# febrianrachmadi/dep-gan-im

Hardware: AMD Instinct MI355X
Metric: 2D slices/sec (G+2D+GP train step), 256x256x1 fp32 (higher is better)
Workload: dtype f32; 1 GPU; DEP-GAN-IM twoCritics canonical train step (critic-Y2 + critic-DEM + G update, WGAN-GP), batch 32 per GPU, 256x256x1; per_gpu_batch=32, global_batch=32, parallelism=dp1

## Files before the change

dep_gan_im_amd/csrc/common.h:

```cpp
#pragma once
#include <hip/hip_runtime.h>
#include <stdint.h>
#include <stddef.h>

typedef float f32x2 __attribute__((ext_vector_type(2)));
typedef float f32x4 __attribute__((ext_vector_type(4)));
typedef float f32x16 __attribute__((ext_vector_type(16)));

struct TView {
  float* p;
  long sB, sY, sX;
};

static inline TView make_view(float* p, int H, int W, int C) {
  TView v;
  v.p = p;
  v.sX = C;
  v.sY = (long)W * C;
  v.sB = (long)H * W * C;
  return v;
}
static inline TView make_view_slice(float* p, int H, int W, int Ctot, int c0) {
  TView v = make_view(p, H, W, Ctot);
  v.p = p + c0;
// ... 32 lines not shown
}

struct Epilogue {
  const float* bias;
  const float* scale;
  const float* shift;
  const float* film_mul;
  const float* film_add;
  int film_ld;
  TView out_pre;
  TView res;
  TView mask;
  int relu;
  int accumulate;
  TView pool;
  const float* head_w;
  const float* head_b;
  float* head_out;
  int head_tanh, head_skip_out;
};

struct ConvArgs {
  TView in;
  TView out;
  const float* w;
  int B, H, W, Cin, Cout;
  Epilogue ep;
  long wsT, wsI, wsO;
  int flip;
  int vec4;
// ... 238 lines not shown
```

dep_gan_im_amd/csrc/igemm_epilogue.inc:

```
#ifndef EPI_PRE_SYNC
#define EPI_PRE_SYNC __syncthreads()
#define EPI_PRE_SYNC_DEFAULTED
#endif
  EPI_PRE_SYNC;
  constexpr int CP = NT + 4;
#ifdef EPI_ES_BASE
  float* es = EPI_ES_BASE;
#else
  float* es = smem + wv * (64 * CP);
#endif
  constexpr int NQ = (MF == 32) ? 4 : 1, CSTEP = (MF == 32) ? 8 : 4;
#if defined(EPI_STAGE)
  EPI_STAGE;
  (void)es;
#elif !defined(EPI_PHASED)
#pragma unroll
  for (int mt = 0; mt < MT; ++mt)
#pragma unroll
    for (int g = 0; g < NQ; ++g) {
      f32x4 q4;
#pragma unroll
      for (int k = 0; k < 4; ++k) q4[k] = acc[mt][4 * g + k];
      *reinterpret_cast<f32x4*>(es + (MF * mt + r) * CP + CSTEP * g + 4 * h) = q4;
    }
// ... 56 lines not shown
      const unsigned lo = __builtin_amdgcn_readfirstlane((unsigned)u), hi = __builtin_amdgcn_readfirstlane((unsigned)(u >> 32));
      return __builtin_amdgcn_make_buffer_rsrc((void*)(((unsigned long long)hi << 32) | lo), 0, 0x7FFFFFFF, 0x00020000);
    };
    const int lo_out = 4 * (pl0 * (int)a.out.sX + co);
    const int lo_pre = has_pre ? 4 * (pl0 * (int)e.out_pre.sX + co) : 0;
    const int lo_res = has_res ? 4 * (pl0 * (int)e.res.sX + co) : 0;
    const int lo_msk = has_msk ? 4 * (pl0 * (int)e.mask.sX + co) : 0;
    const __amdgpu_buffer_rsrc_t r_out = mk(a.out.p + out_goff + view_off(a.out, b, oyw, tx0));
    const __amdgpu_buffer_rsrc_t r_pre = mk(has_pre ? e.out_pre.p + view_off(e.out_pre, b, oyw, tx0) : a.out.p);
    const __amdgpu_buffer_rsrc_t r_res = mk(has_res ? e.res.p + view_off(e.res, b, oyw, tx0) : a.out.p);
    const __amdgpu_buffer_rsrc_t r_msk = mk(has_msk ? e.mask.p + view_off(e.mask, b, oyw, tx0) : a.out.p);
    const __amdgpu_buffer_rsrc_t r_pool =
        mk(has_pool ? e.pool.p + view_off(e.pool, b, oyw >> 1, tx0 >> 1) : a.out.p);
    const int lo_pool = has_pool ? 4 * ((pl0 >> 1) * (int)e.pool.sX + co) : 0;
    const int sY_pool = 4 * (int)e.pool.sY, sX_pool = 4 * (int)e.pool.sX;
    f32x4 vrow = {0.f, 0.f, 0.f, 0.f};
#ifdef EPI_HEAD
#ifdef EPI_CLASS
    const bool has_head = EPI_HEAD && (EPI_CT ? EpiC::head : (e.head_out != nullptr));
#else
    const bool has_head = EPI_HEAD && e.head_out != nullptr;
#endif
    f32x4 hw4 = {0.f, 0.f, 0.f, 0.f};
    if (has_head) hw4 = *reinterpret_cast<const f32x4*>(e.head_w + co);
    const bool skip_out = has_head && e.head_skip_out != 0;
#else
    constexpr bool has_head = false, skip_out = false;
#endif
    typedef int i32x4 __attribute__((ext_vector_type(4)));
    auto ld = [&](const __amdgpu_buffer_rsrc_t& r, int voff, int soff) {
// ... 82 lines not shown
#undef EPI_DPP
        hkeep_out = ((lane & 7) == p) ? d : hkeep_out;
      }
#endif
      if (has_pool) {
        if ((py & 1) == 0) {
          vrow = v;
        } else {
          f32x4 m;
#pragma unroll
          for (int k = 0; k < 4; ++k) {
            const float t = dg_vmax(vrow[k], v[k]);
            m[k] = dg_vmax(t, __shfl_xor(t, LPP, 64));
          }
          if (ok && (pl0 & 1) == 0) st(r_pool, lo_pool, (py >> 1) * sY_pool + (px0 >> 1) * sX_pool, m);
        }
      }
    }
  }
#ifdef EPI_HEAD
  if (EPI_HEAD && a.ep.head_out != nullptr && n0 < a.Cout) {
    const int ph = lane & 7, plh = lane >> 3;
    const int pyh = (ph & 1) + 2 * (ph >> 2), pxh = ((ph >> 1) & 1) * 8 + plh;
    const int yh = oyw + pyh, xh = tx0 + pxh;
    if (yh < a.H && xh < a.W) {
      const float t = hkeep_out + a.ep.head_b[0];
      a.ep.head_out[((long)b * a.H + yh) * a.W + xh] = a.ep.head_tanh ? tanhf(t) : t;
    }
  }
#endif
// ... 5 lines not shown
```

dep_gan_im_amd/csrc/model.h:

```cpp
#pragma once
#include <string.h>

#include <map>
#include <string>
#include <type_traits>
#include <vector>

#include "../../include/depgan.h"
#include "common.h"
#include "bf16s.h"
#include "bf16s_train.h"
#include "deconv_fwd.h"
#include "noise.h"
#include "ops.h"
#include "train_ops.h"

struct PInfo {
  std::string name;
  int shape[4];
  int ndim;
  size_t off, size;
  bool trainable;
};

// ... 41 lines not shown
  int col_mul = -1, col_add = -1;
  TView in, out;
  TViewH hin = null_view_h(), hout = null_view_h(), hu = null_view_h();
  unsigned char* hdec = nullptr;
  int cat_deconv = -1;
  TView din, dout;
  TView in_mask;
  Tn u;
  Tn raw;
  float *bmean = nullptr, *bvar = nullptr, *bs = nullptr, *bt = nullptr, *brstd = nullptr;
  float *cA = nullptr, *cB = nullptr, *cC = nullptr, *sums = nullptr;
  int skip_of = -1;
  TView pool_dsrc;
  TView pool_skipgrad;
  TView pool_dst;
};

struct DLayer {
  std::string name;
  int KS, Cin, Cout, H, W;
  bool pool;
  ConvPlan pf, pb;
  ConvPlan pf16, pb16;
  bool has16f = false, has16b = false;
};

struct DNet {
  Net net;
  PackJob* pack_jobs = nullptr;
  int n_pack = 0;
// ... 38 lines not shown
  float* dheads = nullptr;
  Tn attr;
  Tn du_tmp;
  float* dpre = nullptr;
  float* zbuf = nullptr;

  DNet d[2];
  std::vector<DLayer> dl;
  int NB3 = 0;
  float* d_in = nullptr;
  Tn d_act[11];
  Tn d_pool[11];
  Tn d_dz[11];
  Tn d_dpool[11];
  Tn d_ufull;
  float *d_t9 = nullptr, *d_out = nullptr;
  float* g0 = nullptr;
  float* coefs = nullptr;
  float *norms = nullptr, *gp = nullptr;

  depgan_allreduce_fn ar_fn = nullptr;
  void* ar_user = nullptr;
  int world = 1;
  void* rccl_comm = nullptr;
  long rccl_issued = 0;
  int device = 0;
  bool winograd = true;
  bool head_fused = true;
  bool wgrad_bf16 = true;
  float* host_stats = nullptr;
// ... 42 lines not shown
  float *n_dl = nullptr, *n_dflat = nullptr, *n_dl1 = nullptr, *n_da0 = nullptr, *n_dl0 = nullptr;

  bool dbg_capture = false;
  float* dbg_mixed[11] = {nullptr, nullptr, nullptr, nullptr, nullptr, nullptr, nullptr, nullptr, nullptr, nullptr, nullptr};
  bool dbg_mixed_valid = false;

  bool h_ready = false, h_valid = false;
  bool fwd_only_bf16 = false;
  bool bf16s_head_fused = true;
  bool h_17_skipped = false;
  bool g_update_bf16 = false;
  bool hu_ready = false, hu_valid = false;

  bool critic16_bf16 = false;

  bool prof_on = false;
  std::vector<ProfRec> recs;
};

struct ProfScope {
  depgan_ctx* c;
  bool live;
  ProfScope(depgan_ctx* c_, int klass, double flops, const char* label = "", double bytes = 0.0,
            const char* kernel = "")
      : c(c_), live(c_ && c_->prof_on) {
    if (!live) return;
    ProfRec r;
    r.klass = klass;
    r.flops = flops;
    r.bytes = bytes;
// ... 184 lines not shown
```

dep_gan_im_amd/csrc/model.hip:

```cpp
#include "model.h"

#include <dlfcn.h>
#include <float.h>
#include <math.h>
#include <stdlib.h>
#include <stdarg.h>
#include <stdio.h>
#include <string.h>

static thread_local char g_err[1024] = "";
void dg_set_error(const char* fmt, ...) {
  va_list ap;
  va_start(ap, fmt);
  vsnprintf(g_err, sizeof(g_err), fmt, ap);
  va_end(ap);
}
const char* dg_get_error() { return g_err; }

void Net::add(const std::string& name, std::vector<int> shape, bool trainable) {
  PInfo pi;
  pi.name = name;
  pi.ndim = (int)shape.size();
  pi.size = 1;
  for (int i = 0; i < 4; ++i) {
// ... 447 lines not shown
      L.dout = d.view();
      if (r.per_sample() > maxFilm) maxFilm = r.per_sample();
      cur = L.out;
    } else if (e.kind == G_POOL) {
      const GLayer& Pc = c->gl[i - 1];
      Cat& ct = cats[e.name];
      Tn p, dp;
      DGCHECK(talloc(c, &p, B, H / 2, W / 2, Pc.Cout));
      DGCHECK(galloc(&dp, B, H / 2, W / 2, Pc.Cout));
      L.Cin = L.Cout = Pc.Cout;
      L.skip_of = i - 1;
      L.out = p.view();
      L.pool_dsrc = dp.view();
      L.pool_skipgrad = fwd_only ? null_view() : ct.grad.slice(ct.co_deconv);
      L.pool_dst = Pc.dout;
      H /= 2;
      W /= 2;
      cur = L.out;
    } else if (e.kind == G_DECONV) {
      L.pf = plan_conv(c, 1, L.Cin, L.Cout);
      L.pb = plan_conv(c, 1, L.Cout, L.Cin);
      for (int t = 0; t < 4; ++t) {
        DGCHECK(dmalloc(c, &L.wpf[t], L.pf.packedFloats));
        if (!fwd_only) DGCHECK(dmalloc(c, &L.wpb[t], L.pb.packedFloats));
      }
      L.pbf = plan_conv(c, 1, 4 * L.Cout, L.Cin);
      if (!fwd_only && dg_plan_mfma(L.pb) && L.pbf.family == L.pb.family && L.pbf.planes == L.pb.planes && (L.Cout % L.pb.CK) == 0 &&
          L.pbf.packedFloats == 4 * L.pb.packedFloats)
        DGCHECK(dmalloc(c, &L.wpb_all, L.pbf.packedFloats));
      Cat& ct = cats[e.aux];
// ... 45 lines not shown
    L.H = H;
    L.W = W;
    L.pf = plan_conv(c, L.KS, L.Cin, L.Cout, 96, H, W);
    L.pb = plan_conv(c, L.KS, L.Cout, L.Cin, 96, H, W);
    if (c->cfg.bf16_mfma) {
      L.pf16 = dg_plan_conv_bf16_n16(L.KS, L.Cin, L.Cout);
      L.pb16 = dg_plan_conv_bf16_n16(L.KS, L.Cout, L.Cin);
      L.has16f = dg_plan_mfma(L.pf) && !dg_plan_bf16(L.pf) && dg_plan_bf16(L.pf16);
      L.has16b = l > 0 && dg_plan_mfma(L.pb) && !dg_plan_bf16(L.pb) && dg_plan_bf16(L.pb16);
    }
    DGCHECK(talloc(c, &c->d_act[l], c->NB3, H, W, L.Cout));
    DGCHECK(talloc(c, &c->d_dz[l], c->NB3, H, W, L.Cout));
    if (L.pool) {
      DGCHECK(talloc(c, &c->d_pool[l], c->NB3, H / 2, W / 2, L.Cout));
      DGCHECK(talloc(c, &c->d_dpool[l], c->NB3, H / 2, W / 2, L.Cout));
      H /= 2;
      W /= 2;
    }
  }
  const int HW = H * W;
  DGCHECK(talloc(c, &c->d_ufull, B, H0, W0, 16));
  DGCHECK(dmalloc(c, &c->d_in, (size_t)c->NB3 * H0 * W0));
  DGCHECK(dmalloc(c, &c->d_t9, (size_t)c->NB3 * HW));
  DGCHECK(dmalloc(c, &c->d_out, (size_t)c->NB3));
  DGCHECK(dmalloc(c, &c->g0, (size_t)2 * B * H0 * W0));
  DGCHECK(dmalloc(c, &c->coefs, 8));
  DGCHECK(dmalloc(c, &c->norms, (size_t)B));
  DGCHECK(dmalloc(c, &c->gp, 4));
  const float hc[4] = {-1.0f / B, 1.0f / B, 1.0f, 1.0f};
  HIPCHECK(hipMemcpy(c->coefs, hc, sizeof(hc), hipMemcpyHostToDevice));
// ... 130 lines not shown
        jobs.push_back(j);
      }
      if (D.wpb16[l]) {
        DGCHECK(dg_pack_job(L.pb16, D.W[l], L.Cin, L.Cout, 0, 1, 1, nullptr, D.wpb16[l], 0, &j));
        jobs.push_back(j);
      }
    }
    D.n_pack = (int)jobs.size();
    D.pack_blocks = dg_pack_layout(jobs.data(), D.n_pack);
    DGCHECK(upload_table(c, jobs, &D.pack_jobs));
  }
  ProfScope ps(c, 2, 0.0, "pack weights");
  return dg_pack_weights_batch(D.pack_jobs, D.n_pack, D.pack_blocks, c->st);
}

int g_forward(depgan_ctx* c, const float* x, const float* z, int n, bool store_u) {
  {
    ProfScope ps(c, 2, 0.0, "noise mlp fwd");
    DGCHECK(dg_noise_fwd(c->np, z, c->na, n, c->st));
  }
  bool pooled_by_conv = false, head_by_conv = false;
  for (size_t i = 0; i < c->gl.size(); ++i) {
    GLayer& L = c->gl[i];
    if (L.kind == G_CONV || L.kind == G_FILM) {
      ConvArgs a = conv_args((i == 0) ? make_view(const_cast<float*>(x), L.H, L.W, L.Cin) : L.in, L.out,
                             n, L.H, L.W, L.Cin, L.Cout);
      g_layer_epilogue(&a.ep, L, c->na.heads, L.in);
      if (L.kind == G_FILM && store_u) a.ep.out_pre = L.u.view();
      conv_set_weights(&a, L.pf, L.wpf[0], L.Wt, L.Cin, L.Cout);
      if (dg_plan_mfma(L.pf) && g_pool_follows(c->gl, i)) a.ep.pool = c->gl[i + 1].out;
      pooled_by_conv = a.ep.pool.p != nullptr;
      head_by_conv = false;
      if (L.kind == G_CONV && i + 1 < c->gl.size() && c->gl[i + 1].kind == G_HEAD && c->cfg.nc_out == 1 &&
          c->head_fused && dg_conv_igemm_head_supported(L.pf, a)) {
        const GLayer& Hd = c->gl[i + 1];
        a.ep.head_w = Hd.Wt; a.ep.head_b = Hd.b; a.ep.head_out = c->attr.p;
        a.ep.head_tanh = 1;
        a.ep.head_skip_out = (!store_u && !c->dbg_capture) ? 1 : 0;
        head_by_conv = true;
      }
      DGCHECK(conv_launch(c, L.pf, a, 3));
    } else if (L.kind == G_POOL) {
      if (pooled_by_conv && L.skip_of == (int)i - 1) continue;
      ProfScope ps(c, 2, 0.0, "maxpool");
      DGCHECK(dg_maxpool(c->gl[L.skip_of].out, L.out, n, L.H / 2, L.W / 2, L.Cout, c->st));
// ... 37 lines not shown
      DGCHECK(dg_sum(c->dpre, (size_t)P, L.db, c->scratch, c->scratchFloats, c->st));
      DGCHECK(dg_head_bwd(c->dpre, L.Wt, L.in.p, L.din.p, P, L.Cin, c->st));
    } else if (L.kind == G_CONV) {
      DGCHECK(g_conv_bn_bwd(c, L, (size_t)i, x, L.dout, null_view(), n));
    } else if (L.kind == G_FILM) {
      TView du = make_view(c->du_tmp.p, L.H, L.W, L.Cout);
      {
        ProfScope ps(c, 2, 0.0, "film bwd");
        DGCHECK(dg_film_bwd(L.dout.p, L.u.p, c->na.heads + L.col_mul, c->na.heads + L.col_add, 1024, du.p,
                            c->dheads + L.col_mul, c->dheads + L.col_add, n, (long)L.H * L.W, L.Cout, c->scratch,
                            c->scratchFloats, c->st));
      }
      DGCHECK(g_conv_bn_bwd(c, L, (size_t)i, x, du, L.dout, n));
    } else if (L.kind == G_POOL) {
      ProfScope ps(c, 2, 0.0, "unpool+mask");
      DGCHECK(dg_unpool_mask(L.pool_dsrc, c->gl[L.skip_of].out, L.pool_skipgrad, L.pool_dst, n, L.H / 2, L.W / 2,
                             L.Cout, c->st));
    } else if (L.kind == G_DECONV) {
      DGCHECK(deconv_wgrad_all(c, L, L.in, L.dout, n, L.s, c->raw_all + (L.dW - c->g.G), L.s, L.db, L.dbeta));
      DGCHECK(deconv_bwd_data(c, L, L.dout, n));
    }
  }
  return g_backward_finish(c, z, n);
}

int g_backward_finish(depgan_ctx* c, const float* z, int n) {
  {
    if (!c->g_gamma_jobs) {
      std::vector<GammaJob> jobs;
      int blk = 0;
      for (size_t i = 0; i < c->gl.size(); ++i) {
        const GLayer& L = c->gl[i];
// ... 20 lines not shown
}

static const ConvPlan& d_plan_f(const depgan_ctx* c, int l) {
  return (c->critic16_bf16 && c->dl[l].has16f) ? c->dl[l].pf16 : c->dl[l].pf;
}
static const float* d_panel_f(const depgan_ctx* c, const DNet& D, int l) {
  return (c->critic16_bf16 && c->dl[l].has16f) ? D.wpf16[l] : D.wpf[l];
}
static const ConvPlan& d_plan_b(const depgan_ctx* c, int l) {
  return (c->critic16_bf16 && c->dl[l].has16b) ? c->dl[l].pb16 : c->dl[l].pb;
}
static const float* d_panel_b(const depgan_ctx* c, const DNet& D, int l) {
  return (c->critic16_bf16 && c->dl[l].has16b) ? D.wpb16[l] : D.wpb[l];
}

static int d_forward(depgan_ctx* c, DNet& D, const float* img, long s0, int N) {
  const int H0 = c->cfg.height, W0 = c->cfg.width;
  for (int l = 0; l < 11; ++l) {
    const DLayer& L = c->dl[l];
    ConvArgs a = conv_args((l == 0) ? make_view(const_cast<float*>(img), H0, W0, 1) : d_in_view(c, l, s0),
                           view_offset(c->d_act[l].view(), s0), N, L.H, L.W, L.Cin, L.Cout);
    a.ep.bias = D.b[l];
    a.ep.relu = 1;
    const ConvPlan& pf = d_plan_f(c, l);
    conv_set_weights(&a, pf, d_panel_f(c, D, l), D.W[l], L.Cin, L.Cout);
    if (dg_plan_mfma(pf) && L.pool && !((L.H | L.W) & 1))
      a.ep.pool = view_offset(c->d_pool[l].view(), s0);
    DGCHECK(conv_launch(c, pf, a, L.KS));
    if (L.pool && !a.ep.pool.p) {
      ProfScope ps(c, 2, 0.0, "maxpool");
      DGCHECK(dg_maxpool(a.out, view_offset(c->d_pool[l].view(), s0), N, L.H / 2, L.W / 2, L.Cout, c->st));
    }
  }
  const DLayer& T = c->dl[10];
  const int HW = T.H * T.W;
  ProfScope ps(c, 2, 0.0, "critic tail fwd");
  return dg_critic_tail_fwd(c->d_act[10].p + s0 * c->d_act[10].per_sample(), D.w9, D.b9, D.wd, D.bd,
                            c->d_t9 + s0 * HW, c->d_out + s0, N, HW, 256, c->st);
}

static int d_backward_chain(depgan_ctx* c, DNet& D, long s0, int N, const float* coefs, int per, long img_s0,
                            int img_n, float* g0_out) {
// ... 6 lines not shown
  }
  for (int l = 10; l >= 1; --l) {
    const DLayer& L = c->dl[l];
    const DLayer& Pv = c->dl[l - 1];
    ConvArgs a = conv_args(view_offset(c->d_dz[l].view(), s0), null_view(), N, L.H, L.W, L.Cout, L.Cin);
    a.w = d_panel_b(c, D, l);
    if (Pv.pool) {
      a.out = view_offset(c->d_dpool[l - 1].view(), s0);
    } else {
      a.out = view_offset(c->d_dz[l - 1].view(), s0);
      a.ep.mask = view_offset(c->d_act[l - 1].view(), s0);
    }
    DGCHECK(conv_launch(c, d_plan_b(c, l), a, L.KS));
    if (Pv.pool) {
      ProfScope ps(c, 2, 0.0, "unpool+mask");
      DGCHECK(dg_unpool_mask(a.out, view_offset(c->d_act[l - 1].view(), s0), null_view(),
                             view_offset(c->d_dz[l - 1].view(), s0), N, Pv.H / 2, Pv.W / 2, Pv.Cout, c->st));
    }
  }
  if (img_n > 0) {
    const DLayer& L = c->dl[0];
    ConvArgs a = conv_args(view_offset(c->d_dz[0].view(), s0 + img_s0), make_view(g0_out, L.H, L.W, 1),
                           img_n, L.H, L.W, L.Cout, 1);
    conv_set_weights_bwd(&a, dg_plan_direct(), nullptr, D.W[0], L.Cin, L.Cout);
    DGCHECK(conv_launch(c, dg_plan_direct(), a, L.KS));
  }
  return DG_OK;
}

int net_adam(depgan_ctx* c, Net& n, float gscale) {
  n.adam_t += 1;
  const double b1 = c->cfg.beta1, b2 = c->cfg.beta2;
// ... 30 lines not shown
  n.decay_bits = (unsigned*)b;
  n.gnorm = (double*)g;
  return dalloc_fills_done();
}

static int critic_enqueue(depgan_ctx* c, int which, const float* y2, const float* x, const float* z, const float* ep) {
  if (c->cfg.nc_out != 1) { dg_set_error("the WGAN-GP closures need nc_out == 1"); return DG_ERR_ARG; }
  DNet& D = c->d[which];
  const int B = c->cfg.batch, H0 = c->cfg.height, W0 = c->cfg.width;
  const long HW0 = (long)H0 * W0;
  DGCHECK(g_forward_only(c, x, z));
  {
    ProfScope ps(c, 2, 0.0, "critic inputs");
    DGCHECK(dg_critic_inputs(y2, x, c->cfg.nicg, c->attr.p, ep, c->d_in, B, HW0, which, c->st));
  }
  DGCHECK(d_forward(c, D, c->d_in, 0, 3 * B));
  if (c->dbg_capture) {
    for (int l = 0; l < 11; ++l) {
      const size_t per = c->d_act[l].per_sample();
      if (!c->dbg_mixed[l]) {
        DGCHECK(dmalloc(c, &c->dbg_mixed[l], (size_t)B * per));
        DGCHECK(dalloc_fills_done());
      }
      HIPCHECK(hipMemcpyAsync(c->dbg_mixed[l], c->d_act[l].p + (size_t)2 * B * per, (size_t)B * per * sizeof(float),
                              hipMemcpyDeviceToDevice, c->st));
    }
    c->dbg_mixed_valid = true;
  }
  DGCHECK(d_backward_chain(c, D, 0, 3 * B, c->coefs, B, 2 * B, B, c->g0));
  float* u0 = c->d_in + 2 * B * HW0;
  {
    ProfScope ps(c, 2, 0.0, "gp norms+u0");
    DGCHECK(dg_gp_u0(c->g0, u0, c->norms, nullptr, c->cfg.delta, B, HW0, c->scratch, c->scratchFloats, c->st));
  }
  for (int l = 0; l < 11; ++l) {
    const DLayer& L = c->dl[l];
    TView act = view_offset(c->d_act[l].view(), 2 * B);
    ConvArgs a = conv_args((l == 0) ? make_view(u0, H0, W0, 1) : d_in_view(c, l, 2 * B),
                           L.pool ? make_view(c->d_ufull.p, L.H, L.W, L.Cout) : act, B, L.H, L.W, L.Cin, L.Cout);
    a.ep.mask = act;
    conv_set_weights(&a, d_plan_f(c, l), d_panel_f(c, D, l), D.W[l], L.Cin, L.Cout);
    DGCHECK(conv_launch(c, d_plan_f(c, l), a, L.KS));
    if (L.pool) {
      ProfScope ps(c, 2, 0.0, "gather pool");
      DGCHECK(dg_gather_pool(a.out, act, view_offset(c->d_pool[l].view(), 2 * B), B, L.H / 2, L.W / 2, L.Cout,
                             c->st));
    }
  }
  for (int l = 0; l < 11; ++l) {
    const DLayer& L = c->dl[l];
    TView xin = (l == 0) ? make_view(c->d_in, H0, W0, 1) : d_in_view(c, l, 0);
    const ColSum cs = {2 * B, nullptr, D.db[l], nullptr};
    DGCHECK(wgrad_full(c, L.KS, xin, c->d_dz[l].view(), 3 * B, L.H, L.W, L.Cin, L.Cout, nullptr, D.dW[l], nullptr, 0,
                       0, &cs));
  }
  {
    ProfScope ps(c, 2, 0.0, "critic tail wgrad+stats");
    const DLayer& T = c->dl[10];
    const int HW = T.H * T.W;
    DGCHECK(dg_critic_tail_wgrad(c->d_act[10].p, D.w9, D.b9, D.wd, c->coefs, B, 1, 0, D.dw9, D.db9, D.dwd, D.dbd,
                                 c->scratch, c->scratchFloats, 2 * B, HW, 256, c->st));
// ... 7 lines not shown

static int g_eval_enqueue(depgan_ctx* c, const float* x, const float* y2, const float* z, bool train,
                          float* stats_dev) {
  const int B = c->cfg.batch, H0 = c->cfg.height, W0 = c->cfg.width;
  const long HW0 = (long)H0 * W0, P = (long)B * HW0;
  if (train) {
    if (c->g_update_bf16) DGCHECK(g_forward_train_bf16s(c, x, z));
    else DGCHECK(g_forward(c, x, z, B, true));
  } else {
    DGCHECK(g_forward_only(c, x, z));
  }
  {
    ProfScope ps(c, 2, 0.0, "fake_y2");
    DGCHECK(dg_add_ch0(x, c->cfg.nicg, c->attr.p, c->fake_y2, P, c->st));
  }
  DGCHECK(d_forward(c, c->d[0], c->fake_y2, 0, B));
  DGCHECK(d_forward(c, c->d[1], c->attr.p, B, B));
  {
    ProfScope ps(c, 2, 0.0, "g loss sums");
    DGCHECK(dg_sum_groups_consts(c->d_out, stats_dev, 2, B, 6, (float)B, (float)P, c->st));
    DGCHECK(dg_gloss_sums(x, c->cfg.nicg, y2, c->attr.p, c->cfg.im_thresh, stats_dev + 2, P, c->scratch,
                                  c->scratchFloats, c->st));
  }
  if (train) {
    DGCHECK(d_backward_chain(c, c->d[0], 0, B, c->coefs + 2, B, 0, B, c->g0));
    DGCHECK(d_backward_chain(c, c->d[1], B, B, c->coefs + 2, B, 0, B, c->g0 + P));
    {
      ProfScope ps(c, 2, 0.0, "g dpre");
      DGCHECK(dg_g_dpre(x, c->cfg.nicg, y2, c->attr.p, c->g0, c->g0 + P, c->dpre, B, P, c->st));
    }
    if (c->g_update_bf16) DGCHECK(g_backward_bf16s(c, x, z, B));
    else DGCHECK(g_backward(c, x, z, B));
// ... 167 lines not shown
    dg_set_error("depgan_create: need batch >= 1, height/width multiples of 16, nicg in {1,2}");
    return DG_ERR_ARG;
  }
  depgan_ctx* c = new depgan_ctx();
  c->cfg = *cfg;
  if (hipGetDevice(&c->device) != hipSuccess) c->device = 0;
  {
    const char* e = getenv("DEPGAN_WGRAD_BF16");
    c->wgrad_bf16 = !(e && atoi(e) == 0);
    const char* hf = getenv("DEPGAN_HEAD_FUSED");
    c->head_fused = !(hf && atoi(hf) == 0);
    const char* hfs = getenv("DEPGAN_BF16S_HEAD_FUSED");
    c->bf16s_head_fused = !(hfs && atoi(hfs) == 0);
    const char* wn = getenv("DEPGAN_WINOGRAD");
    c->winograd = !(wn && atoi(wn) == 0);
  }
  if (c->cfg.nc_out == 0) c->cfg.nc_out = 1;
  if (c->cfg.nc_out < 1 || c->cfg.nc_out > DEPGAN_MAX_HEAD_CLASSES) {
    dg_set_error("depgan_create: nc_out must be 1 (DEP-GAN) or in [2, %d] (DEP-UResNet classes), not %d",
                 DEPGAN_MAX_HEAD_CLASSES, c->cfg.nc_out);
    delete c;
    return DG_ERR_ARG;
  }
  c->infer_only = c->cfg.bf16_mfma && c->cfg.nc_out >= 2;
  c->train_bn = c->cfg.nc_out != 1 && !c->infer_only;
  memset(c->last_sums, 0, sizeof(c->last_sums));
  int rc = build_generator(c);
  if (rc == DG_OK && !c->train_bn && !c->infer_only) rc = build_critics(c);
  if (rc == DG_OK && c->train_bn) rc = uresnet_build(c);
  if (rc == DG_OK && c->infer_only)
// ... 204 lines not shown
  if (pipe != 0 && pipe != 1) {
    dg_set_error("depgan_set_critic16_pipe: pipe must be 0 (fp32) or 1 (bf16), got %d", pipe);
    return DG_ERR_ARG;
  }
  DGCHECK(infer_refuse(c, "depgan_set_critic16_pipe"));
  if (pipe == 1 && (!c->cfg.bf16_mfma || c->dl.empty())) {
    dg_set_error("depgan_set_critic16_pipe: the bf16 pipe for the critics' 16-channel layers needs a context created with "
                 "bf16_mfma = 1 (and critics: nc_out = 1)");
    return DG_ERR_UNSUPPORTED;
  }
  c->critic16_bf16 = pipe == 1;
  return DG_OK;
}
int depgan_get_critic16_pipe(depgan_ctx* c) { return (c && c->critic16_bf16) ? 1 : 0; }

int depgan_g_forward(depgan_ctx* c, const float* x, const float* z, float* out, int n) {
  if (n < 1 || n > c->cfg.batch) { dg_set_error("g_forward: n must be in [1, batch]"); return DG_ERR_ARG; }
  if (c->cfg.nc_out != 1) return uresnet_predict(c, x, z, out, n);
  DGCHECK(g_forward(c, x, z, n, false));
  HIPCHECK(hipMemcpyAsync(out, c->attr.p, (size_t)n * c->cfg.height * c->cfg.width * sizeof(float),
                          hipMemcpyDeviceToDevice, c->st));
  return DG_OK;
}

int depgan_d_forward(depgan_ctx* c, int net, const float* img, float* out, int n) {
  DGCHECK(infer_refuse(c, "depgan_d_forward"));
  if (net != DEPGAN_NET_D_Y2 && net != DEPGAN_NET_D_DEM) { dg_set_error("d_forward: not a critic id"); return DG_ERR_ARG; }
  if (n < 1 || n > c->NB3) { dg_set_error("d_forward: n must be in [1, 3*batch]"); return DG_ERR_ARG; }
  DGCHECK(d_forward(c, c->d[net - 1], img, 0, n));
  HIPCHECK(hipMemcpyAsync(out, c->d_out, (size_t)n * sizeof(float), hipMemcpyDeviceToDevice, c->st));
  return DG_OK;
}

int depgan_critic_grads(depgan_ctx* c, int net, const float* y2, const float* x, const float* z, const float* ep,
                        float out[2]) {
  return critic_impl(c, net, y2, x, z, ep, out, false);
}

int depgan_apply_adam(depgan_ctx* c, int net) {
  DGCHECK(infer_refuse(c, "depgan_apply_adam"));
  Net* n = pick_net(c, net);
  if (!n) return DG_ERR_ARG;
  DGCHECK(net_adam(c, *n));
  return depgan_weights_changed(c, net);
// ... 236 lines not shown
    const std::string ln = want_u ? rest("g/u/") : rest("g/out/");
    for (const GLayer& L : c->gl) {
      if (L.name != ln) continue;
      if (want_u) {
        if (L.kind != G_FILM || !L.u.p) break;
        v = L.u.view();
        H = L.H; W = L.W;
      } else {
        v = L.out;
        H = L.kind == G_POOL ? L.H / 2 : (L.kind == G_DECONV ? 2 * L.H : L.H);
        W = L.kind == G_POOL ? L.W / 2 : (L.kind == G_DECONV ? 2 * L.W : L.W);
      }
      N = B; C = L.Cout;
      break;
    }
  } else if (starts("d/act/") || starts("d/mixed/")) {
    const bool mixed = starts("d/mixed/");
    const std::string ln = mixed ? rest("d/mixed/") : rest("d/act/");
    for (size_t l = 0; l < c->dl.size(); ++l) {
      if (c->dl[l].name != ln) continue;
      if (mixed) {
        if (!c->dbg_mixed_valid || !c->dbg_mixed[l]) { dg_set_error("debug_tensor: %s was not captured (depgan_debug_capture)", name); return DG_ERR_ARG; }
        v = make_view(c->dbg_mixed[l], c->dl[l].H, c->dl[l].W, c->dl[l].Cout);
        N = B;
      } else {
        v = c->d_act[l].view();
        N = c->NB3;
      }
      H = c->dl[l].H; W = c->dl[l].W; C = c->dl[l].Cout;
      break;
// ... 24 lines not shown
```

dep_gan_im_amd/csrc/ops.h:

```cpp
#pragma once
#include "common.h"

int dg_maxpool(TView in, TView out, int B, int Ho, int Wo, int C, hipStream_t st);
int dg_unpool_mask(TView dpool, TView a, TView skip , TView out, int B, int Ho, int Wo, int C,
                   hipStream_t st);
int dg_gather_pool(TView u, TView a, TView out, int B, int Ho, int Wo, int C, hipStream_t st);

int dg_bn_prepare(const float* gamma, const float* beta, const float* mean, const float* var, float eps, float* s,
                  float* t, float* rstd, int C, hipStream_t st);

int dg_head_fwd(const float* a, const float* w, const float* b, float* out, long P, int C, int tanh_act,
                hipStream_t st);
int dg_head_bwd(const float* dpre, const float* w, const float* a, float* dz, long P, int C, hipStream_t st);

int dg_critic_tail_fwd(const float* a, const float* w9, const float* b9, const float* wd, const float* bd, float* t9,
                       float* out, int N, int HW, int C, hipStream_t st);
int dg_critic_tail_bwd(const float* a, const float* w9, const float* wd, const float* coefs, int per, float* dz, int N,
                       int HW, int C, hipStream_t st);
int dg_critic_tail_wgrad(const float* src, const float* w9, const float* b9, const float* wd, const float* coefs,
                         int per, int add_bias_terms, int accumulate, float* dw9, float* db9, float* dwd, float* dbd,
                         float* scratch, size_t scratch_floats, int N, int HW, int C, hipStream_t st);
size_t dg_critic_tail_wgrad_scratch(int N, int HW, int C);

struct BnJob {
// ... 66 lines not shown
```

dep_gan_im_amd/csrc/ops.hip:

```cpp
#include "ops.h"
#include <float.h>
#include <hip/hip_bf16.h>
#include "epilogue.h"

__device__ __forceinline__ float wave_sum(float v) {
#pragma unroll
  for (int o = 32; o > 0; o >>= 1) v += __shfl_down(v, o, 64);
  return v;
}
__device__ __forceinline__ float block_sum(float v, float* sh4) {
  v = wave_sum(v);
  __syncthreads();
  if ((threadIdx.x & 63) == 0) sh4[threadIdx.x >> 6] = v;
  __syncthreads();
  return (sh4[0] + sh4[1]) + (sh4[2] + sh4[3]);
}

static inline int nblk(size_t n, int cap = 2048) {
  size_t b = (n + 255) / 256;
  return (int)(b > (size_t)cap ? cap : (b < 1 ? 1 : b));
}

static int scratch_ok(const char* who, size_t need, size_t have) {
  if (need <= have) return 1;
// ... 102 lines not shown
}

int dg_unpool_mask(TView dpool, TView a, TView skip, TView out, int B, int Ho, int Wo, int C, hipStream_t st) {
  if (C % 4) { dg_set_error("dg_unpool_mask: C %% 4 != 0"); return DG_ERR_ARG; }
  const size_t total = (size_t)B * Ho * Wo * (C / 4);
  hipLaunchKernelGGL(pool_bwd_kernel<0>, dim3(nblk(total, 8192)), dim3(256), 0, st, dpool, a, skip, out, B, Ho, Wo,
                     C / 4);
  HIPCHECK(hipGetLastError());
  return DG_OK;
}
int dg_gather_pool(TView u, TView a, TView out, int B, int Ho, int Wo, int C, hipStream_t st) {
  if (C % 4) { dg_set_error("dg_gather_pool: C %% 4 != 0"); return DG_ERR_ARG; }
  const size_t total = (size_t)B * Ho * Wo * (C / 4);
  hipLaunchKernelGGL(pool_bwd_kernel<1>, dim3(nblk(total, 8192)), dim3(256), 0, st, u, a, null_view(), out, B, Ho,
                     Wo, C / 4);
  HIPCHECK(hipGetLastError());
  return DG_OK;
}

__global__ void bn_prepare_kernel(const float* gamma, const float* beta, const float* mean, const float* var,
                                  float eps, float* s, float* t, float* rstd, int C) {
  const int c = blockIdx.x * blockDim.x + threadIdx.x;
  if (c >= C) return;
  const float r = 1.0f / sqrtf(var[c] + eps);
  const float sc = gamma[c] * r;
  s[c] = sc;
  t[c] = beta[c] - mean[c] * sc;
  rstd[c] = r;
}
int dg_bn_prepare(const float* gamma, const float* beta, const float* mean, const float* var, float eps, float* s,
// ... 961 lines not shown
```

dep_gan_im_amd/engine.py:

```python
from __future__ import annotations

import ctypes as C
import os
from collections import OrderedDict

import numpy as np

from . import _lib
from ._lib import (ARENA_ADAM_M, ARENA_ADAM_V, ARENA_GRADS, ARENA_NONTRAINABLE, ARENA_PARAMS, D2H, H2D, NET_D_DEM,
                   NET_D_Y2, NET_G, Config, check, load)

NET_IDS = {"G": NET_G, "D_y2": NET_D_Y2, "D_dem": NET_D_DEM}
_DICE_FORMS = {"flat": _lib._K["DEPGAN_DICE_FLAT"], "class": _lib._K["DEPGAN_DICE_CLASS"]}


def _torch():
    import torch
    return torch


def require_class_indices(labels):
    torch = _torch()
    tens = isinstance(labels, torch.Tensor)
    a = labels if tens else np.asarray(labels)
# ... 266 lines not shown

    @property
    def critic16_pipe(self):
        return getattr(self, "_critic16_pipe", "float32")

    @critic16_pipe.setter
    def critic16_pipe(self, value):
        if value not in ("float32", "bfloat16"):
            raise ValueError("critic16_pipe must be 'float32' or 'bfloat16', got %r" % (value,))
        self._need_trainable("critic16_pipe")
        if value == "bfloat16" and not (self.cfg.bf16_mfma and self.cfg.nc_out in (0, 1)):
            raise ValueError("critic16_pipe='bfloat16' needs an engine created with bf16_mfma=True (and nc_out=1); "
                             "this one has bf16_mfma=%d, nc_out=%d" % (self.cfg.bf16_mfma, self.cfg.nc_out))
        self._set_mode("critic16_pipe", "depgan_set_critic16_pipe", value)

    def g_forward(self, x, z, storage=None):
        storage = self.forward_storage if storage is None else self._check_storage(storage)
        torch = _torch()
        x = self._dev(x)
        z = self._dev(z).reshape(x.shape[0], -1)
        if x.dim() != 4 or tuple(x.shape[1:]) != (self.height, self.width, self.nicg):
            raise ValueError("generator input must be (N,%d,%d,%d), got %s" % (self.height, self.width, self.nicg,
                                                                                tuple(x.shape)))
        if z.shape[1] != 32:
            raise ValueError("noise input must be (N,32,1)")
        n = x.shape[0]
        out = torch.empty((n, self.height, self.width, self.nc_out), dtype=torch.float32, device=self.device)
        self._use_current_stream()
        fn, what = ((self.lib.depgan_g_forward_bf16s, "depgan_g_forward_bf16s") if storage == "bfloat16"
                    else (self.lib.depgan_g_forward, "depgan_g_forward"))
# ... 375 lines not shown
```

include/depgan.h:

```cpp
#ifndef DEPGAN_H
#define DEPGAN_H
#include <stddef.h>
#ifdef __cplusplus
extern "C" {
#endif

typedef struct depgan_ctx depgan_ctx;

#define DEPGAN_ABI_VERSION 3
int depgan_abi_version(void);
size_t depgan_config_size(void);
const char* depgan_source_hash(void);

typedef struct depgan_config {
  int struct_size;
  int batch;
  int height;
  int width;
  int nicg;
  int first_fm;
  float im_thresh;
  float delta;
  float lrD, lrG;
  float beta1, beta2, adam_eps;
// ... 167 lines not shown

int depgan_debug_capture(depgan_ctx* ctx, int on);
int depgan_debug_tensor(depgan_ctx* ctx, const char* name, float* host_dst, long cap_floats, int shape[4]);

int depgan_g_forward_bf16s(depgan_ctx* ctx, const float* x_dev, const float* z_dev, float* out_dev, int n);
int depgan_debug_tensor_bf16s(depgan_ctx* ctx, const char* name, float* host_dst, long cap_floats, int shape[4]);

int depgan_set_fwd_only_storage(depgan_ctx* ctx, int storage);
int depgan_get_fwd_only_storage(depgan_ctx* ctx);

int depgan_set_g_update_storage(depgan_ctx* ctx, int storage);
int depgan_get_g_update_storage(depgan_ctx* ctx);

int depgan_set_critic16_pipe(depgan_ctx* ctx, int pipe);
int depgan_get_critic16_pipe(depgan_ctx* ctx);
int depgan_debug_film_decision_bf16s(depgan_ctx* ctx, const char* layer, unsigned char* host_dst, long cap_bytes,
                                     int shape[4]);

int depgan_op_conv2d_film_train_bf16s(const void* in, long isB, long isY, long isX, const float* w_hwio, const float* bias,
                                      const float* scale, const float* shift, const float* film_mul, const float* film_add,
                                      int film_ld, const void* res, long rsB, long rsY, long rsX, void* out, long osB,
                                      long osY, long osX, void* u_out, unsigned char* dec_bits, int B, int H, int W, int Cin,
                                      int Cout, int relu, void* hip_stream);
int depgan_op_conv2d_wgrad_bf16s(const void* x, long xsB, long xsY, long xsX, const float* dy, long dsB, long dsY, long dsX,
                                 float* dw, float* colsum, int B, int H, int W, int Cin, int Cout, int KS, int oi,
                                 void* hip_stream);
int depgan_op_conv2d_bwd_data_bf16s(const float* dy, long dsB, long dsY, long dsX, const float* w, const float* res,
                                    long rsB, long rsY, long rsX, const void* mask, long msB, long msY, long msX, float* dx,
                                    long osB, long osY, long osX, int B, int H, int W, int Cin, int Cout, int deconv,
                                    void* hip_stream);
// ... 186 lines not shown
```

Baseline: 714.4 slices/s.

## Record maxpool argmax and ReLU codes in conv epilogue for backward unpool

```diff
diff --git a/dep_gan_im_amd/csrc/common.h b/dep_gan_im_amd/csrc/common.h
--- a/dep_gan_im_amd/csrc/common.h
+++ b/dep_gan_im_amd/csrc/common.h
@@ -70,6 +70,7 @@
   int relu;
   int accumulate;
   TView pool;
+  unsigned char* pool_code;
   const float* head_w;
   const float* head_b;
   float* head_out;
diff --git a/dep_gan_im_amd/csrc/igemm_epilogue.inc b/dep_gan_im_amd/csrc/igemm_epilogue.inc
--- a/dep_gan_im_amd/csrc/igemm_epilogue.inc
+++ b/dep_gan_im_amd/csrc/igemm_epilogue.inc
@@ -94,6 +94,9 @@
         mk(has_pool ? e.pool.p + view_off(e.pool, b, oyw >> 1, tx0 >> 1) : a.out.p);
     const int lo_pool = has_pool ? 4 * ((pl0 >> 1) * (int)e.pool.sX + co) : 0;
     const int sY_pool = 4 * (int)e.pool.sY, sX_pool = 4 * (int)e.pool.sX;
+    const bool has_code = has_pool && e.pool_code != nullptr;
+    unsigned char* const p_code =
+        has_code ? e.pool_code + (view_off(e.pool, b, oyw >> 1, tx0 >> 1) + (pl0 >> 1) * (int)e.pool.sX + co) : nullptr;
     f32x4 vrow = {0.f, 0.f, 0.f, 0.f};
 #ifdef EPI_HEAD
 #ifdef EPI_CLASS
@@ -206,6 +209,24 @@
             m[k] = dg_vmax(t, __shfl_xor(t, LPP, 64));
           }
           if (ok && (pl0 & 1) == 0) st(r_pool, lo_pool, (py >> 1) * sY_pool + (px0 >> 1) * sX_pool, m);
+          if (has_code) {
+            unsigned mine = 0;
+#pragma unroll
+            for (int k = 0; k < 4; ++k) {
+              const unsigned f = (vrow[k] == m[k] ? 1u : 0u) | (v[k] == m[k] ? 2u : 0u) | (vrow[k] > 0.f ? 4u : 0u) |
+                                 (v[k] > 0.f ? 8u : 0u);
+              mine |= f << (8 * k);
+            }
+            const unsigned oth = (unsigned)__shfl_xor((int)mine, LPP, 64);
+            constexpr unsigned B0 = 0x01010101u;
+            const unsigned ne0 = ~mine & B0;
+            const unsigned am0 = ne0 & (oth | ~(mine >> 1));
+            const unsigned am1 = ne0 & ~oth;
+            const unsigned code = am0 | (am1 << 1) | (mine & (B0 << 2)) | ((oth & (B0 << 2)) << 1) |
+                                  ((mine & (B0 << 3)) << 1) | ((oth & (B0 << 3)) << 2);
+            if (ok && (pl0 & 1) == 0)
+              *reinterpret_cast<unsigned*>(p_code + (((py >> 1) * sY_pool + (px0 >> 1) * sX_pool) >> 2)) = code;
+          }
         }
       }
     }
diff --git a/dep_gan_im_amd/csrc/model.h b/dep_gan_im_amd/csrc/model.h
--- a/dep_gan_im_amd/csrc/model.h
+++ b/dep_gan_im_amd/csrc/model.h
@@ -79,6 +79,7 @@
   TView pool_dsrc;
   TView pool_skipgrad;
   TView pool_dst;
+  unsigned char* pool_code = nullptr;
 };
 
 struct DLayer {
@@ -147,6 +148,7 @@
   Tn d_dz[11];
   Tn d_dpool[11];
   Tn d_ufull;
+  unsigned char* d_code[11] = {nullptr, nullptr, nullptr, nullptr, nullptr, nullptr, nullptr, nullptr, nullptr, nullptr, nullptr};
   float *d_t9 = nullptr, *d_out = nullptr;
   float* g0 = nullptr;
   float* coefs = nullptr;
@@ -219,6 +221,8 @@
 
   bool critic16_bf16 = false;
 
+  bool pool_codes = true;
+
   bool prof_on = false;
   std::vector<ProfRec> recs;
 };
diff --git a/dep_gan_im_amd/csrc/model.hip b/dep_gan_im_amd/csrc/model.hip
--- a/dep_gan_im_amd/csrc/model.hip
+++ b/dep_gan_im_amd/csrc/model.hip
@@ -485,6 +485,11 @@
       L.pool_dsrc = dp.view();
       L.pool_skipgrad = fwd_only ? null_view() : ct.grad.slice(ct.co_deconv);
       L.pool_dst = Pc.dout;
+      if (!fwd_only && c->cfg.nc_out < 2) {
+        void* cp = nullptr;
+        HIPCHECK(dalloc_bytes(c, &cp, (size_t)B * (H / 2) * (W / 2) * Pc.Cout));
+        L.pool_code = static_cast<unsigned char*>(cp);
+      }
       H /= 2;
       W /= 2;
       cur = L.out;
@@ -560,6 +565,9 @@
     if (L.pool) {
       DGCHECK(talloc(c, &c->d_pool[l], c->NB3, H / 2, W / 2, L.Cout));
       DGCHECK(talloc(c, &c->d_dpool[l], c->NB3, H / 2, W / 2, L.Cout));
+      void* cp = nullptr;
+      HIPCHECK(dalloc_bytes(c, &cp, (size_t)c->NB3 * (H / 2) * (W / 2) * L.Cout));
+      c->d_code[l] = static_cast<unsigned char*>(cp);
       H /= 2;
       W /= 2;
     }
@@ -720,6 +728,12 @@
   return dg_pack_weights_batch(D.pack_jobs, D.n_pack, D.pack_blocks, c->st);
 }
 
+static unsigned char* g_pool_codes(const depgan_ctx* c, size_t ip) {
+  const GLayer& L = c->gl[ip];
+  if (!c->pool_codes || !L.pool_code || ip == 0 || L.skip_of != (int)ip - 1) return nullptr;
+  return (dg_plan_mfma(c->gl[ip - 1].pf) && g_pool_follows(c->gl, ip - 1)) ? L.pool_code : nullptr;
+}
+
 int g_forward(depgan_ctx* c, const float* x, const float* z, int n, bool store_u) {
   {
     ProfScope ps(c, 2, 0.0, "noise mlp fwd");
@@ -734,7 +748,10 @@
       g_layer_epilogue(&a.ep, L, c->na.heads, L.in);
       if (L.kind == G_FILM && store_u) a.ep.out_pre = L.u.view();
       conv_set_weights(&a, L.pf, L.wpf[0], L.Wt, L.Cin, L.Cout);
-      if (dg_plan_mfma(L.pf) && g_pool_follows(c->gl, i)) a.ep.pool = c->gl[i + 1].out;
+      if (dg_plan_mfma(L.pf) && g_pool_follows(c->gl, i)) {
+        a.ep.pool = c->gl[i + 1].out;
+        if (store_u) a.ep.pool_code = g_pool_codes(c, i + 1);
+      }
       pooled_by_conv = a.ep.pool.p != nullptr;
       head_by_conv = false;
       if (L.kind == G_CONV && i + 1 < c->gl.size() && c->gl[i + 1].kind == G_HEAD && c->cfg.nc_out == 1 &&
@@ -802,8 +819,11 @@
       DGCHECK(g_conv_bn_bwd(c, L, (size_t)i, x, du, L.dout, n));
     } else if (L.kind == G_POOL) {
       ProfScope ps(c, 2, 0.0, "unpool+mask");
-      DGCHECK(dg_unpool_mask(L.pool_dsrc, c->gl[L.skip_of].out, L.pool_skipgrad, L.pool_dst, n, L.H / 2, L.W / 2,
-                             L.Cout, c->st));
+      if (const unsigned char* code = g_pool_codes(c, (size_t)i))
+        DGCHECK(dg_unpool_codes(L.pool_dsrc, code, L.pool_skipgrad, L.pool_dst, n, L.H / 2, L.W / 2, L.Cout, c->st));
+      else
+        DGCHECK(dg_unpool_mask(L.pool_dsrc, c->gl[L.skip_of].out, L.pool_skipgrad, L.pool_dst, n, L.H / 2, L.W / 2,
+                               L.Cout, c->st));
     } else if (L.kind == G_DECONV) {
       DGCHECK(deconv_wgrad_all(c, L, L.in, L.dout, n, L.s, c->raw_all + (L.dW - c->g.G), L.s, L.db, L.dbeta));
       DGCHECK(deconv_bwd_data(c, L, L.dout, n));
@@ -854,7 +874,13 @@
   return (c->critic16_bf16 && c->dl[l].has16b) ? D.wpb16[l] : D.wpb[l];
 }
 
-static int d_forward(depgan_ctx* c, DNet& D, const float* img, long s0, int N) {
+static unsigned char* d_pool_codes(const depgan_ctx* c, int l, long s0) {
+  const DLayer& L = c->dl[l];
+  if (!c->pool_codes || !L.pool || !c->d_code[l] || ((L.H | L.W) & 1) || !dg_plan_mfma(d_plan_f(c, l))) return nullptr;
+  return c->d_code[l] + s0 * ((long)(L.H / 2) * (L.W / 2) * L.Cout);
+}
+
+static int d_forward(depgan_ctx* c, DNet& D, const float* img, long s0, int N, bool codes) {
   const int H0 = c->cfg.height, W0 = c->cfg.width;
   for (int l = 0; l < 11; ++l) {
     const DLayer& L = c->dl[l];
@@ -866,6 +892,7 @@
     conv_set_weights(&a, pf, d_panel_f(c, D, l), D.W[l], L.Cin, L.Cout);
     if (dg_plan_mfma(pf) && L.pool && !((L.H | L.W) & 1))
       a.ep.pool = view_offset(c->d_pool[l].view(), s0);
+    if (a.ep.pool.p && codes) a.ep.pool_code = d_pool_codes(c, l, s0);
     DGCHECK(conv_launch(c, pf, a, L.KS));
     if (L.pool && !a.ep.pool.p) {
       ProfScope ps(c, 2, 0.0, "maxpool");
@@ -902,8 +929,12 @@
     DGCHECK(conv_launch(c, d_plan_b(c, l), a, L.KS));
     if (Pv.pool) {
       ProfScope ps(c, 2, 0.0, "unpool+mask");
-      DGCHECK(dg_unpool_mask(a.out, view_offset(c->d_act[l - 1].view(), s0), null_view(),
-                             view_offset(c->d_dz[l - 1].view(), s0), N, Pv.H / 2, Pv.W / 2, Pv.Cout, c->st));
+      TView dz = view_offset(c->d_dz[l - 1].view(), s0);
+      if (const unsigned char* code = d_pool_codes(c, l - 1, s0))
+        DGCHECK(dg_unpool_codes(a.out, code, null_view(), dz, N, Pv.H / 2, Pv.W / 2, Pv.Cout, c->st));
+      else
+        DGCHECK(dg_unpool_mask(a.out, view_offset(c->d_act[l - 1].view(), s0), null_view(), dz, N, Pv.H / 2, Pv.W / 2,
+                               Pv.Cout, c->st));
     }
   }
   if (img_n > 0) {
@@ -964,7 +995,7 @@
     ProfScope ps(c, 2, 0.0, "critic inputs");
     DGCHECK(dg_critic_inputs(y2, x, c->cfg.nicg, c->attr.p, ep, c->d_in, B, HW0, which, c->st));
   }
-  DGCHECK(d_forward(c, D, c->d_in, 0, 3 * B));
+  DGCHECK(d_forward(c, D, c->d_in, 0, 3 * B, true));
   if (c->dbg_capture) {
     for (int l = 0; l < 11; ++l) {
       const size_t per = c->d_act[l].per_sample();
@@ -993,8 +1024,11 @@
     DGCHECK(conv_launch(c, d_plan_f(c, l), a, L.KS));
     if (L.pool) {
       ProfScope ps(c, 2, 0.0, "gather pool");
-      DGCHECK(dg_gather_pool(a.out, act, view_offset(c->d_pool[l].view(), 2 * B), B, L.H / 2, L.W / 2, L.Cout,
-                             c->st));
+      TView up = view_offset(c->d_pool[l].view(), 2 * B);
+      if (const unsigned char* code = d_pool_codes(c, l, 2 * B))
+        DGCHECK(dg_gather_codes(a.out, code, up, B, L.H / 2, L.W / 2, L.Cout, c->st));
+      else
+        DGCHECK(dg_gather_pool(a.out, act, up, B, L.H / 2, L.W / 2, L.Cout, c->st));
     }
   }
   for (int l = 0; l < 11; ++l) {
@@ -1032,8 +1066,8 @@
     ProfScope ps(c, 2, 0.0, "fake_y2");
     DGCHECK(dg_add_ch0(x, c->cfg.nicg, c->attr.p, c->fake_y2, P, c->st));
   }
-  DGCHECK(d_forward(c, c->d[0], c->fake_y2, 0, B));
-  DGCHECK(d_forward(c, c->d[1], c->attr.p, B, B));
+  DGCHECK(d_forward(c, c->d[0], c->fake_y2, 0, B, train));
+  DGCHECK(d_forward(c, c->d[1], c->attr.p, B, B, train));
   {
     ProfScope ps(c, 2, 0.0, "g loss sums");
     DGCHECK(dg_sum_groups_consts(c->d_out, stats_dev, 2, B, 6, (float)B, (float)P, c->st));
@@ -1231,6 +1265,8 @@
     c->bf16s_head_fused = !(hfs && atoi(hfs) == 0);
     const char* wn = getenv("DEPGAN_WINOGRAD");
     c->winograd = !(wn && atoi(wn) == 0);
+    const char* pc = getenv("DEPGAN_POOL_CODES");
+    c->pool_codes = !(pc && atoi(pc) == 0);
   }
   if (c->cfg.nc_out == 0) c->cfg.nc_out = 1;
   if (c->cfg.nc_out < 1 || c->cfg.nc_out > DEPGAN_MAX_HEAD_CLASSES) {
@@ -1465,6 +1501,14 @@
 }
 int depgan_get_critic16_pipe(depgan_ctx* c) { return (c && c->critic16_bf16) ? 1 : 0; }
 
+int depgan_set_pool_codes(depgan_ctx* c, int on) {
+  if (!c) { dg_set_error("depgan_set_pool_codes: null context"); return DG_ERR_ARG; }
+  if (on != 0 && on != 1) { dg_set_error("depgan_set_pool_codes: on must be 0 or 1, got %d", on); return DG_ERR_ARG; }
+  c->pool_codes = on == 1;
+  return DG_OK;
+}
+int depgan_get_pool_codes(depgan_ctx* c) { return (c && c->pool_codes) ? 1 : 0; }
+
 int depgan_g_forward(depgan_ctx* c, const float* x, const float* z, float* out, int n) {
   if (n < 1 || n > c->cfg.batch) { dg_set_error("g_forward: n must be in [1, batch]"); return DG_ERR_ARG; }
   if (c->cfg.nc_out != 1) return uresnet_predict(c, x, z, out, n);
@@ -1478,7 +1522,7 @@
   DGCHECK(infer_refuse(c, "depgan_d_forward"));
   if (net != DEPGAN_NET_D_Y2 && net != DEPGAN_NET_D_DEM) { dg_set_error("d_forward: not a critic id"); return DG_ERR_ARG; }
   if (n < 1 || n > c->NB3) { dg_set_error("d_forward: n must be in [1, 3*batch]"); return DG_ERR_ARG; }
-  DGCHECK(d_forward(c, c->d[net - 1], img, 0, n));
+  DGCHECK(d_forward(c, c->d[net - 1], img, 0, n, false));
   HIPCHECK(hipMemcpyAsync(out, c->d_out, (size_t)n * sizeof(float), hipMemcpyDeviceToDevice, c->st));
   return DG_OK;
 }
@@ -1745,6 +1789,40 @@
       N = B; C = L.Cout;
       break;
     }
+  } else if (starts("g/din/") || starts("g/code/")) {
+    const bool code = starts("g/code/");
+    const std::string ln = code ? rest("g/code/") : rest("g/din/");
+    for (const GLayer& L : c->gl) {
+      if (L.name != ln) continue;
+      if (code) {
+        if (L.kind != G_POOL || !L.pool_code) break;
+        v = make_view(reinterpret_cast<float*>(L.pool_code), L.H / 2, L.W / 2, L.Cout / 4);
+        H = L.H / 2; W = L.W / 2; C = L.Cout / 4;
+      } else {
+        if (!L.din.p) break;
+        v = L.din;
+        H = L.H; W = L.W; C = L.Cin;
+      }
+      N = B;
+      break;
+    }
+  } else if (starts("d/dz/") || starts("d/code/")) {
+    const bool code = starts("d/code/");
+    const std::string ln = code ? rest("d/code/") : rest("d/dz/");
+    for (size_t l = 0; l < c->dl.size(); ++l) {
+      const DLayer& L = c->dl[l];
+      if (L.name != ln) continue;
+      if (code) {
+        if (!c->d_code[l]) break;
+        v = make_view(reinterpret_cast<float*>(c->d_code[l]), L.H / 2, L.W / 2, L.Cout / 4);
+        H = L.H / 2; W = L.W / 2; C = L.Cout / 4;
+      } else {
+        v = c->d_dz[l].view();
+        H = L.H; W = L.W; C = L.Cout;
+      }
+      N = c->NB3;
+      break;
+    }
   } else if (starts("d/act/") || starts("d/mixed/")) {
     const bool mixed = starts("d/mixed/");
     const std::string ln = mixed ? rest("d/mixed/") : rest("d/act/");
diff --git a/dep_gan_im_amd/csrc/ops.h b/dep_gan_im_amd/csrc/ops.h
--- a/dep_gan_im_amd/csrc/ops.h
+++ b/dep_gan_im_amd/csrc/ops.h
@@ -5,6 +5,9 @@
 int dg_unpool_mask(TView dpool, TView a, TView skip , TView out, int B, int Ho, int Wo, int C,
                    hipStream_t st);
 int dg_gather_pool(TView u, TView a, TView out, int B, int Ho, int Wo, int C, hipStream_t st);
+int dg_unpool_codes(TView dpool, const unsigned char* code, TView skip , TView out, int B, int Ho, int Wo,
+                    int C, hipStream_t st);
+int dg_gather_codes(TView u, const unsigned char* code, TView out, int B, int Ho, int Wo, int C, hipStream_t st);
 
 int dg_bn_prepare(const float* gamma, const float* beta, const float* mean, const float* var, float eps, float* s,
                   float* t, float* rstd, int C, hipStream_t st);
diff --git a/dep_gan_im_amd/csrc/ops.hip b/dep_gan_im_amd/csrc/ops.hip
--- a/dep_gan_im_amd/csrc/ops.hip
+++ b/dep_gan_im_amd/csrc/ops.hip
@@ -140,6 +140,97 @@
   const size_t total = (size_t)B * Ho * Wo * (C / 4);
   hipLaunchKernelGGL(pool_bwd_kernel<1>, dim3(nblk(total, 8192)), dim3(256), 0, st, u, a, null_view(), out, B, Ho,
                      Wo, C / 4);
+  HIPCHECK(hipGetLastError());
+  return DG_OK;
+}
+
+__global__ void unpool_codes_kernel(TView d, const unsigned char* __restrict__ code, TView skip, TView out, int B,
+                                    int Ho, int Wo, int C4) {
+  const size_t total = (size_t)B * Ho * Wo * C4;
+  for (size_t i = blockIdx.x * (size_t)blockDim.x + threadIdx.x; i < total; i += (size_t)gridDim.x * blockDim.x) {
+    size_t q = i;
+    const int c = (int)(q % C4) * 4;
+    q /= C4;
+    const int x = (int)(q % Wo);
+    q /= Wo;
+    const int y = (int)(q % Ho);
+    const int b = (int)(q / Ho);
+    const unsigned cw = *reinterpret_cast<const unsigned*>(code + 4 * i);
+    const f32x4 dv = *reinterpret_cast<const f32x4*>(d.p + view_off(d, b, y, x) + c);
+    f32x4 o[4];
+#pragma unroll
+    for (int w = 0; w < 4; ++w) o[w] = (f32x4){0.f, 0.f, 0.f, 0.f};
+    if (skip.p) {
+      const float* ps = skip.p + view_off(skip, b, 2 * y, 2 * x) + c;
+      o[0] = *reinterpret_cast<const f32x4*>(ps);
+      o[1] = *reinterpret_cast<const f32x4*>(ps + skip.sX);
+      o[2] = *reinterpret_cast<const f32x4*>(ps + skip.sY);
+      o[3] = *reinterpret_cast<const f32x4*>(ps + skip.sY + skip.sX);
+    }
+#pragma unroll
+    for (int k = 0; k < 4; ++k) {
+      const unsigned ck = cw >> (8 * k);
+      const int am = (int)(ck & 3u);
+#pragma unroll
+      for (int w = 0; w < 4; ++w) {
+        float v = o[w][k] + ((w == am) ? dv[k] : 0.f);
+        o[w][k] = ((ck >> (2 + w)) & 1u) ? v : 0.f;
+      }
+    }
+    float* po = out.p + view_off(out, b, 2 * y, 2 * x) + c;
+    *reinterpret_cast<f32x4*>(po) = o[0];
+    *reinterpret_cast<f32x4*>(po + out.sX) = o[1];
+    *reinterpret_cast<f32x4*>(po + out.sY) = o[2];
+    *reinterpret_cast<f32x4*>(po + out.sY + out.sX) = o[3];
+  }
+}
+
+__global__ void gather_codes_kernel(TView u, const unsigned char* __restrict__ code, TView out, int B, int Ho, int Wo,
+                                    int C4) {
+  const size_t total = (size_t)B * Ho * Wo * C4;
+  for (size_t i = blockIdx.x * (size_t)blockDim.x + threadIdx.x; i < total; i += (size_t)gridDim.x * blockDim.x) {
+    size_t q = i;
+    const int c = (int)(q % C4) * 4;
+    q /= C4;
+    const int x = (int)(q % Wo);
+    q /= Wo;
+    const int y = (int)(q % Ho);
+    const int b = (int)(q / Ho);
+    const unsigned cw = *reinterpret_cast<const unsigned*>(code + 4 * i);
+    const float* pu = u.p + view_off(u, b, 2 * y, 2 * x) + c;
+    f32x4 uv[4];
+    uv[0] = *reinterpret_cast<const f32x4*>(pu);
+    uv[1] = *reinterpret_cast<const f32x4*>(pu + u.sX);
+    uv[2] = *reinterpret_cast<const f32x4*>(pu + u.sY);
+    uv[3] = *reinterpret_cast<const f32x4*>(pu + u.sY + u.sX);
+    f32x4 o;
+#pragma unroll
+    for (int k = 0; k < 4; ++k) {
+      const int am = (int)((cw >> (8 * k)) & 3u);
+      o[k] = (am == 0) ? uv[0][k] : (am == 1) ? uv[1][k] : (am == 2) ? uv[2][k] : uv[3][k];
+    }
+    *reinterpret_cast<f32x4*>(out.p + view_off(out, b, y, x) + c) = o;
+  }
+}
+
+static int codes_args_ok(const char* who, const unsigned char* code, int C) {
+  if (!code || ((uintptr_t)code & 3)) { dg_set_error("%s: the code buffer must be non-null and 4-byte aligned", who); return 0; }
+  if (C % 4) { dg_set_error("%s: C %% 4 != 0", who); return 0; }
+  return 1;
+}
+int dg_unpool_codes(TView dpool, const unsigned char* code, TView skip, TView out, int B, int Ho, int Wo, int C,
+                    hipStream_t st) {
+  if (!codes_args_ok("dg_unpool_codes", code, C)) return DG_ERR_ARG;
+  const size_t total = (size_t)B * Ho * Wo * (C / 4);
+  hipLaunchKernelGGL(unpool_codes_kernel, dim3(nblk(total, 8192)), dim3(256), 0, st, dpool, code, skip, out, B, Ho, Wo,
+                     C / 4);
+  HIPCHECK(hipGetLastError());
+  return DG_OK;
+}
+int dg_gather_codes(TView u, const unsigned char* code, TView out, int B, int Ho, int Wo, int C, hipStream_t st) {
+  if (!codes_args_ok("dg_gather_codes", code, C)) return DG_ERR_ARG;
+  const size_t total = (size_t)B * Ho * Wo * (C / 4);
+  hipLaunchKernelGGL(gather_codes_kernel, dim3(nblk(total, 8192)), dim3(256), 0, st, u, code, out, B, Ho, Wo, C / 4);
   HIPCHECK(hipGetLastError());
   return DG_OK;
 }
diff --git a/dep_gan_im_amd/engine.py b/dep_gan_im_amd/engine.py
--- a/dep_gan_im_amd/engine.py
+++ b/dep_gan_im_amd/engine.py
@@ -304,6 +304,14 @@
                              "this one has bf16_mfma=%d, nc_out=%d" % (self.cfg.bf16_mfma, self.cfg.nc_out))
         self._set_mode("critic16_pipe", "depgan_set_critic16_pipe", value)
 
+    @property
+    def pool_codes(self):
+        return bool(self.lib.depgan_get_pool_codes(self.h))
+
+    @pool_codes.setter
+    def pool_codes(self, on):
+        check(self.lib.depgan_set_pool_codes(self.h, 1 if on else 0), "depgan_set_pool_codes")
+
     def g_forward(self, x, z, storage=None):
         storage = self.forward_storage if storage is None else self._check_storage(storage)
         torch = _torch()
diff --git a/include/depgan.h b/include/depgan.h
--- a/include/depgan.h
+++ b/include/depgan.h
@@ -205,6 +205,9 @@
 
 int depgan_set_critic16_pipe(depgan_ctx* ctx, int pipe);
 int depgan_get_critic16_pipe(depgan_ctx* ctx);
+
+int depgan_set_pool_codes(depgan_ctx* ctx, int on);
+int depgan_get_pool_codes(depgan_ctx* ctx);
 int depgan_debug_film_decision_bf16s(depgan_ctx* ctx, const char* layer, unsigned char* host_dst, long cap_bytes,
                                      int shape[4]);
 
```

Result: no change. 718.8 slices/s, median of 6 (+0.6%).
